# taohan10200/CRA5

Measured on AMD Instinct MI355X. Metric: ERA5 frames/s (721x1440x268) encode+decode, higher is better.
Workload: dtype f32 (3xf16-split MFMA, fp32 accumulate)

## Files before the change

### cra5_amd/config.py

```python
import dataclasses
import os
from dataclasses import dataclass


def _flag(v):
    return str(v).strip().lower() not in ("0", "false", "off", "no", "")


@dataclass
class RuntimeConfig:
    precision: str = "fp32"
    gemm_engine: str = "split"
    attn_engine: str = "split"
    range_guard: bool = True
    gpu_exclusive: bool = True
    gpu_slots: int = 3
    inflight: int = 12
    switch_interval_s: float = 0.0002
    copy_threads: int = 8
    batch_copy_threads: int = 1
    link_serial: bool = True
    numa_bind_single: bool = True
    weights: str = ""

    ENV = {
        "precision": "CRA5_PRECISION", "gemm_engine": "CRA5_GEMM", "attn_engine": "CRA5_ATTN", "range_guard": "CRA5_RANGE_GUARD",
        "gpu_exclusive": "CRA5_GPU_EXCLUSIVE", "gpu_slots": "CRA5_GPU_SLOTS", "inflight": "CRA5_INFLIGHT",
        "switch_interval_s": "CRA5_SWITCH_INTERVAL", "copy_threads": "CRA5_COPY_THREADS",
        "batch_copy_threads": "CRA5_BATCH_COPY_THREADS", "link_serial": "CRA5_LINK_SERIAL",
        "numa_bind_single": "CRA5_NUMA_BIND_SINGLE", "weights": "CRA5_WEIGHTS",
    }

    def __post_init__(self):
        if self.precision not in ("fp32", "f16"):
            raise ValueError("precision (CRA5_PRECISION) must be 'fp32' or 'f16'")
        if self.gemm_engine not in ("split", "f32"):
            raise ValueError("gemm_engine (CRA5_GEMM) must be 'split' or 'f32'")
        if self.attn_engine not in ("split", "f32"):
            raise ValueError("attn_engine (CRA5_ATTN) must be 'split' or 'f32'")
        if self.gpu_slots < 0 or self.inflight < 1 or not (1 <= self.copy_threads <= 64) or not (1 <= self.batch_copy_threads <= 64):
            raise ValueError("gpu_slots >= 0, inflight >= 1, 1 <= copy threads <= 64")
# ... 33 lines not shown
```

### cra5_amd/csrc/elementwise.hip

```cpp
#include <hip/hip_runtime.h>
#include <math.h>

#include "../../include/cra5_amd.h"
#include "split.h"
#pragma clang force_cuda_host_device begin
#include "rans_resolve.h"
#pragma clang force_cuda_host_device end

CRA5_RANGE_TU(elementwise)
#ifdef CRA5_RANGE_CHECK
extern "C" {
int cra5_range_counts_gemm(unsigned long long *, int);
int cra5_range_counts_attn(unsigned long long *, int);
int cra5_range_counts_attn_f32(unsigned long long *, int);
int cra5_range_counts_hyper(unsigned long long *, int);
}
#endif

namespace {

__device__ __forceinline__ float wave_sum(float v) {
#pragma unroll
  for (int off = 32; off > 0; off >>= 1) v += __shfl_xor(v, off, 64);
  return v;
// ... 47 lines not shown
        if (ys_plain) cra5_store_plain4(ys + (size_t)row * 2 * Kp, c, o.x, o.y, o.z, o.w);
        else cra5_store_split4(ys + (size_t)row * 2 * Kp, c, o.x, o.y, o.z, o.w);
      }
    }
  }
  if (ys)
    for (int c = D + lane; c < Kp; c += 64) {
      if (ys_plain) cra5_store_plain(ys + (size_t)row * 2 * Kp, c, 0.f);
      else cra5_store_split(ys + (size_t)row * 2 * Kp, c, 0.f);
    }
}

__global__ __launch_bounds__(256) void im2col_kernel(const float *__restrict__ x, const float *__restrict__ mean,
                                                     const float *__restrict__ stdv, float *__restrict__ cols,
                                                     unsigned short *__restrict__ cols_s, int C, int H, int W,
                                                     int kh, int kw, int sh, int sw, int Hp, int Wp, int ldk, int plain) {
  const int K = C * kh * kw;
  const size_t total = (size_t)Hp * Wp * K;
  for (size_t e = (size_t)blockIdx.x * blockDim.x + threadIdx.x; e < total; e += (size_t)gridDim.x * blockDim.x) {
    const int tok = (int)(e / K);
    const int k = (int)(e - (size_t)tok * K);
    const int ph = tok / Wp, pw = tok - ph * Wp;
    const int c = k / (kh * kw);
    const int ij = k - c * kh * kw;
    const int i = ij / kw, j = ij - i * kw;
    float v = x[((size_t)c * H + (ph * sh + i)) * W + (pw * sw + j)];
    if (mean) v = (v - mean[c]) / stdv[c];
    if (cols) cols[(size_t)tok * ldk + k] = v;
    if (cols_s) {
      if (plain) cra5_store_plain(cols_s + (size_t)tok * 2 * ldk, k, v);
      else cra5_store_split(cols_s + (size_t)tok * 2 * ldk, k, v);
    }
  }
}

__global__ __launch_bounds__(256) void col2im_kernel(const float *__restrict__ cols, const float *__restrict__ mean,
                                                     const float *__restrict__ stdv, float *__restrict__ x, int C,
                                                     int H, int W, int kh, int kw, int sh, int sw, int Hp, int Wp,
                                                     int ldn) {
  const size_t total = (size_t)C * H * W;
  for (size_t e = (size_t)blockIdx.x * blockDim.x + threadIdx.x; e < total; e += (size_t)gridDim.x * blockDim.x) {
    const int col = (int)(e % W);
    const size_t t = e / W;
    const int row = (int)(t % H);
    const int c = (int)(t / H);
// ... 16 lines not shown
    if (mean) acc = acc * stdv[c] + mean[c];
    x[e] = acc;
  }
}


constexpr int TILE_TOK = 16;
constexpr int TILE_CH = 2;
constexpr int TILE_CH_S = 2;
constexpr int IM2COL_GROUP = 2;

template <int KH, int KW>
__global__ __launch_bounds__(256) void im2col_tiled_kernel(const float *__restrict__ x, const float *__restrict__ mean,
                                                           const float *__restrict__ stdv, float *__restrict__ cols,
                                                           unsigned short *__restrict__ cols_s, int C, int H, int W,
                                                           int sh, int Hp, int Wp, int ldk, int plain) {
  constexpr int SEG = TILE_TOK * KW;
  constexpr int TS = TILE_CH * KH * KW + 4;
  static_assert((TILE_CH * KH * KW) % 4 == 0, "a block's K offset must stay 16-byte aligned");
  constexpr int NL = 4;
  static_assert(TILE_CH * KH * (SEG / 4) <= 256 * NL, "a channel chunk must fit one pass of loads");
  __shared__ __attribute__((aligned(16))) float tile[TILE_TOK * TS];
  const int tiles_w = Wp / TILE_TOK;
  const int n_cc = (C + TILE_CH - 1) / TILE_CH;
  constexpr int G = IM2COL_GROUP;
  const int n_g = (n_cc + G - 1) / G;
  const int g = blockIdx.x % n_g;
  const int pwt = (blockIdx.x / n_g) % tiles_w;
  const int ph = blockIdx.x / (n_g * tiles_w);
  const int col0 = pwt * SEG;
  const int cc_lo = g * G, cc_hi = min(cc_lo + G, n_cc);
// ... 27 lines not shown
        for (int u = 0; u < 4; ++u) vv[u] = (vv[u] - m) / sd;
      }
#pragma unroll
      for (int u = 0; u < 4; ++u) {
        const int col = p4 * 4 + u;
        const int t = col / KW, j = col - t * KW;
        tile[t * TS + row * KW + j] = vv[u];
      }
    }
  }
  __syncthreads();
  if (cc + 1 < cc_hi) load(cc + 1);
  const int kpt = nc * KH * KW;
  const int q4 = (kpt + 3) / 4;
  const int kbase = c0 * KH * KW;
  for (int e = threadIdx.x; e < TILE_TOK * q4; e += 256) {
    const int t = e / q4, k4 = (e - t * q4) * 4;
    const float4 v = *reinterpret_cast<const float4 *>(tile + t * TS + k4);
    const size_t tok = (size_t)ph * Wp + pwt * TILE_TOK + t;
    if (k4 + 4 <= kpt) {
      if (cols) *reinterpret_cast<float4 *>(cols + tok * ldk + kbase + k4) = v;
      if (cols_s) {
        if (plain) cra5_store_plain4(cols_s + tok * 2 * ldk, kbase + k4, v.x, v.y, v.z, v.w);
        else cra5_store_split4(cols_s + tok * 2 * ldk, kbase + k4, v.x, v.y, v.z, v.w);
      }
    } else {
      const float vv[4] = {v.x, v.y, v.z, v.w};
      for (int u = 0; k4 + u < kpt; ++u) {
        if (cols) cols[tok * ldk + kbase + k4 + u] = vv[u];
        if (cols_s) {
          if (plain) cra5_store_plain(cols_s + tok * 2 * ldk, kbase + k4 + u, vv[u]);
          else cra5_store_split(cols_s + tok * 2 * ldk, kbase + k4 + u, vv[u]);
        }
      }
    }
  }
  if (plain && cols_s && cc == n_cc - 1) {
    const int K = C * KH * KW, npad = ldk - K;
    for (int e = threadIdx.x; e < TILE_TOK * npad; e += 256) {
      const int t = e / npad, k = K + (e - t * npad);
      cols_s[((size_t)ph * Wp + pwt * TILE_TOK + t) * 2 * ldk + k] = 0;
    }
  }
  if (cc + 1 < cc_hi) __syncthreads();
  }
}

template <int KH, int KW>
__global__ __launch_bounds__(256) void col2im_tiled_kernel(const float *__restrict__ cols, const float *__restrict__ mean,
                                                           const float *__restrict__ stdv, float *__restrict__ x, int C,
                                                           int H, int W, int sh, int Hp, int Wp, int ldn) {
  constexpr int SEG = TILE_TOK * KW;
// ... 381 lines not shown
#define CRA5_LN(V) hipLaunchKernelGGL(layernorm_kernel<V>, grid, block, 0, st, x, ldx, gamma, beta, y, ldy, y_split, split_kp, rows, D, eps, split_plain)
  if (D <= 256) CRA5_LN(1);
  else if (D <= 512) CRA5_LN(2);
  else if (D <= 1024) CRA5_LN(4);
  else CRA5_LN(8);
#undef CRA5_LN
  return (int)hipGetLastError();
}

int cra5_im2col_f32(const float *x, const float *mean, const float *stdv, float *cols, uint16_t *cols_split, int C,
                    int H, int W, int kh, int kw, int sh, int sw, int Hp, int Wp, int ldk, int split_plain, void *stream) {
  if (!x || (!cols && !cols_split) || C <= 0 || ldk < C * kh * kw) return CRA5_ERR_ARG;
  if (cols_split && (ldk % 32)) return CRA5_ERR_ARG;
  if ((Hp - 1) * sh + kh > H || (Wp - 1) * sw + kw > W) return CRA5_ERR_ARG;
  if ((mean == nullptr) != (stdv == nullptr)) return CRA5_ERR_ARG;
  if (kh == 11 && kw == 10 && sw == 10 && sh == 10 && Wp % TILE_TOK == 0 && (W % 4) == 0 && (ldk % 4) == 0 &&
      ((uintptr_t)x & 15) == 0) {
    const int n_cc = (C + TILE_CH - 1) / TILE_CH;
    const int blocks = (Wp / TILE_TOK) * Hp * ((n_cc + IM2COL_GROUP - 1) / IM2COL_GROUP);
    hipLaunchKernelGGL((im2col_tiled_kernel<11, 10>), dim3(blocks), dim3(256), 0, (hipStream_t)stream, x, mean, stdv,
                       cols, cols_split, C, H, W, sh, Hp, Wp, ldk, split_plain);
    return (int)hipGetLastError();
  }
  if (split_plain && ldk != C * kh * kw) return CRA5_ERR_ARG;
  const size_t total = (size_t)Hp * Wp * C * kh * kw;
  hipLaunchKernelGGL(im2col_kernel, dim3(grid_for(total)), dim3(256), 0, (hipStream_t)stream, x, mean, stdv, cols,
                     cols_split, C, H, W, kh, kw, sh, sw, Hp, Wp, ldk, split_plain);
  return (int)hipGetLastError();
}

int cra5_col2im_f32(const float *cols, const float *mean, const float *stdv, float *x, int C, int H, int W, int kh,
                    int kw, int sh, int sw, int Hp, int Wp, int ldn, void *stream) {
  if (!x || !cols || C <= 0 || ldn < C * kh * kw) return CRA5_ERR_ARG;
  if ((Hp - 1) * sh + kh != H || (Wp - 1) * sw + kw != W) return CRA5_ERR_ARG;
  if ((mean == nullptr) != (stdv == nullptr)) return CRA5_ERR_ARG;
  if (kh == 11 && kw == 10 && sw == 10 && sh == 10 && Wp % TILE_TOK == 0 && (W % 4) == 0 && (ldn % 4) == 0 &&
      ((uintptr_t)cols & 15) == 0 && ((uintptr_t)x & 15) == 0) {
    const int blocks = (Wp / TILE_TOK) * Hp * ((C + TILE_CH_S - 1) / TILE_CH_S);
    hipLaunchKernelGGL((col2im_tiled_kernel<11, 10>), dim3(blocks), dim3(256), 0, (hipStream_t)stream, cols, mean,
                       stdv, x, C, H, W, sh, Hp, Wp, ldn);
    return (int)hipGetLastError();
  }
// ... 155 lines not shown
```

### cra5_amd/csrc/gemm_split_f16.hip

```cpp
#include <hip/hip_runtime.h>
#include <stdlib.h>
#include <type_traits>

#include "../../include/cra5_amd.h"
#include "split.h"

CRA5_RANGE_TU(gemm)

typedef float f32x16 __attribute__((ext_vector_type(16)));
typedef _Float16 half8 __attribute__((ext_vector_type(8)));

namespace {

constexpr int BK = 32;

__device__ __forceinline__ float gelu_erf(float x) {
  const float t = __builtin_fabsf(x) * 0.70710678118654752440f;
  const float k = __builtin_amdgcn_rcpf(__builtin_fmaf(0.4f, t, 1.0f));
  float p = 0.03080804832279682f;
  p = __builtin_fmaf(p, k, -0.3524225652217865f);
  p = __builtin_fmaf(p, k, 1.0205539464950562f);
  p = __builtin_fmaf(p, k, -0.7088391780853271f);
  p = __builtin_fmaf(p, k, 0.6733116507530212f);
  p = __builtin_fmaf(p, k, 0.0958886444568634f);
// ... 35 lines not shown
  if (threadIdx.x == 0 && blockIdx.x < 8192) g_gemm_trace[blockIdx.x * 5 + (slot)] = wall_clock64();
#else
#define CRA5_TRACE(slot)
#endif

struct UnembedArgs {
  float *side;
  const float *mean, *stdv;
  int H, W, Hp, Wp;
};

template <int WM, int WN, int TM, int TN, bool LONGK, int NPROD = 3, bool UE = false>
__global__ __launch_bounds__(WM *WN * 64, ((WM * WN == 4 && TM == 3) ? 2 : 1)) void gemm_nt_split_kernel(
    const unsigned short *__restrict__ A, long lda, const unsigned short *__restrict__ W, long ldw, float *C,
    int ldc, unsigned short *Cs, long ldcs, const float *__restrict__ bias, const float *res, int ldr, int M,
    int N, int Kp, float wscale_inv, int flags, int tiles_n, UnembedArgs ue) {
  constexpr int BM = WM * TM * 32;
  constexpr int BN = WN * TN * 32;
  constexpr int NT = WM * WN * 64;
  constexpr int ROWS_PER_PASS = NT / 8;
  constexpr int A_P = BM / ROWS_PER_PASS;
  constexpr int B_P = BN / ROWS_PER_PASS;
  static_assert(BM % ROWS_PER_PASS == 0 && BN % ROWS_PER_PASS == 0, "tile/threads mismatch");
  constexpr int STAGE = (BM + BN) * 64;

  __shared__ __attribute__((aligned(16))) unsigned short lds[2 * STAGE];

  CRA5_TRACE(0);
#ifdef CRA5_GEMM_TRACE
  if (threadIdx.x == 0 && blockIdx.x < 8192) g_gemm_trace[blockIdx.x * 5 + 4] = clock64();
#endif
// ... 53 lines not shown
        src[q] = W + (size_t)min(n0 + row_, N - 1) * ldw + poffs + (size_t)ka * 64;
      if (ASM_DMA)
        soff[q] = (unsigned)((((size_t)(isA ? (size_t)(min(m0 + row_, M - 1) - m0) * lda : (size_t)(min(n0 + row_, N - 1) - n0) * ldw)) + poffs) * 2);
    }
  }
  if (ASM_DMA) {
    curA = reinterpret_cast<unsigned long long>(A + (size_t)m0 * lda) + (unsigned long long)ka * 128;
    curW = reinterpret_cast<unsigned long long>(W + (size_t)n0 * ldw) + (unsigned long long)ka * 128;
  }
#if defined(__HIP_DEVICE_COMPILE__)
#define CRA5_GLDS16(SRC, DST) __builtin_amdgcn_global_load_lds(SRC, DST, 16, 0, 0)
#else
#define CRA5_GLDS16(SRC, DST) (void)(SRC)
#endif
#define CRA5_DMA_KSTRIDE (2 * KSTEP * 2)
  const unsigned kstride_a = a_plain ? 128u : (unsigned)CRA5_DMA_KSTRIDE, kstride_w = w_plain ? 128u : (unsigned)CRA5_DMA_KSTRIDE;
#if defined(__HIP_DEVICE_COMPILE__)
#define CRA5_STAGE_LOAD(BUF)                                                                   \
  {                                                                                            \
    if (ASM_DMA) {                                                                             \
             \
      const unsigned ldsb_ = (unsigned)(size_t)((__attribute__((address_space(3))) unsigned short *)(lds + (BUF)*STAGE)); \
      _Pragma("unroll") for (int q = 0; q < IPW; ++q) {                                        \
        const unsigned dst_ = ldsb_ + (wave_dma + q * NWAVE) * 1024;                           \
        asm volatile("s_mov_b32 m0, %0\n\ts_nop 0\n\tglobal_load_lds_dwordx4 %1, %2"          \
                     :: "s"(dst_), "v"(soff[q]), "s"((q * NWAVE * 8 < BM) ? curA : curW) : "memory", "m0"); \
      }                                                                                        \
      curA += kstride_a;                                                                       \
      curW += kstride_w;                                                                       \
    } else {                                                                                   \
      _Pragma("unroll") for (int q = 0; q < IPW; ++q) {                                        \
// ... 196 lines not shown

__global__ __launch_bounds__(256) void split_rows_kernel(const float *__restrict__ x, long ldx,
                                                         unsigned short *__restrict__ out, int rows, int K, int Kp,
                                                         float scale) {
  const size_t total = (size_t)rows * Kp;
  for (size_t e = (size_t)blockIdx.x * blockDim.x + threadIdx.x; e < total; e += (size_t)gridDim.x * blockDim.x) {
    const int r = (int)(e / Kp), k = (int)(e - (size_t)r * Kp);
    const float v = (k < K) ? x[(size_t)r * ldx + k] * scale : 0.f;
    cra5_store_split(out + (size_t)r * 2 * Kp, k, v);
  }
}

template <int WM, int WN, int TM, int TN, bool LONGK, int NPROD = 3, bool UE = false>
int launch(const unsigned short *A, long lda, const unsigned short *W, long ldw, float *C, int ldc,
           unsigned short *Cs, long ldcs, const float *bias, const float *res, int ldr, int M, int N, int Kp,
           float wscale_inv, int flags, hipStream_t st, UnembedArgs ue = UnembedArgs{}) {
  constexpr int BM = WM * TM * 32, BN = WN * TN * 32;
  const int tiles_m = (M + BM - 1) / BM, tiles_n = (N + BN - 1) / BN;
  hipLaunchKernelGGL((gemm_nt_split_kernel<WM, WN, TM, TN, LONGK, NPROD, UE>), dim3(tiles_m * tiles_n),
                     dim3(WM * WN * 64), 0, st, A, lda, W, ldw, C, ldc, Cs, ldcs, bias, res, ldr, M, N, Kp, wscale_inv,
                     flags, tiles_n, ue);
  return (int)hipGetLastError();
}

__global__ __launch_bounds__(256) void unembed_fixup_kernel(const float *__restrict__ side, const float *__restrict__ mean,
                                                            const float *__restrict__ stdv, float *__restrict__ x, int C,
                                                            int H, int W, int Hp) {
  const int w4 = W / 4;
  const size_t total = (size_t)C * (Hp + 1) * w4;
  for (size_t e = (size_t)blockIdx.x * blockDim.x + threadIdx.x; e < total; e += (size_t)gridDim.x * blockDim.x) {
    const int p4 = (int)(e % w4);
    const size_t t = e / w4;
    const int i = (int)(t % (Hp + 1)), c = (int)(t / (Hp + 1));
    float4 v = make_float4(0.f, 0.f, 0.f, 0.f);
    bool have = false;
    if (i > 0) {
// ... 4 lines not shown
      const float4 b = *reinterpret_cast<const float4 *>(side + (((size_t)c * Hp + i) * 2 + 0) * W + 4 * p4);
      v = have ? make_float4(v.x + b.x, v.y + b.y, v.z + b.z, v.w + b.w) : b;
    }
    if (mean) {
      const float m = mean[c], sd = stdv[c];
      v = make_float4(v.x * sd + m, v.y * sd + m, v.z * sd + m, v.w * sd + m);
    }
    *reinterpret_cast<float4 *>(x + ((size_t)c * H + (size_t)10 * i) * W + 4 * p4) = v;
  }
}

}

static int gemm_dispatch(const unsigned short *A, long lda, const unsigned short *W, long ldw, float *C, int ldc,
                         unsigned short *C_split, long ldcs, const float *bias, const float *res, int ldr, int M,
                         int N, int Kp, float wscale_inv, int flags, hipStream_t st) {
  const long tiles128 = (long)((M + 127) / 128) * ((N + 127) / 128);
#define CRA5_GO(WM, WN, TM, TN, LK) \
  return launch<WM, WN, TM, TN, LK>(A, lda, W, ldw, C, ldc, C_split, ldcs, bias, res, ldr, M, N, Kp, wscale_inv, flags, st)
#ifdef CRA5_GEMM_TRACE
  static const int forced = [] {
    const char *e = getenv("CRA5_GEMM_TILE");
    return e ? atoi(e) : 0;
  }();
#else
  constexpr int forced = 0;
#endif
  const bool longk = Kp > 8192;
  const bool force_wide = flags & CRA5_GEMM_WIDE_K;
  if (force_wide && (!(flags & CRA5_GEMM_HI_ONLY) || longk || (Kp % 64))) return CRA5_ERR_ARG;
  constexpr int PLAIN_ANY = CRA5_GEMM_A_PLAIN | CRA5_GEMM_W_PLAIN | CRA5_GEMM_OUT_PLAIN;
  if ((flags & PLAIN_ANY) && (!(flags & CRA5_GEMM_HI_ONLY) || longk || (tiles128 < 256 && !force_wide) || (Kp % 64)))
    return CRA5_ERR_ARG;
  if (longk) CRA5_GO(2, 2, 2, 2, true);
  if (flags & CRA5_GEMM_HI_ONLY) {
    const bool wide = (M >= 1024 && N >= 2048);
    if (tiles128 < 256 && !force_wide)
      return launch<2, 2, 1, 1, false, 1>(A, lda, W, ldw, C, ldc, C_split, ldcs, bias, res, ldr, M, N, Kp, wscale_inv, flags, st);
    if (Kp % 64 == 0) {
      if (wide)
        return launch<2, 4, 4, 2, false, 2>(A, lda, W, ldw, C, ldc, C_split, ldcs, bias, res, ldr, M, N, Kp, wscale_inv, flags, st);
      return launch<2, 4, 3, 2, false, 2>(A, lda, W, ldw, C, ldc, C_split, ldcs, bias, res, ldr, M, N, Kp, wscale_inv, flags, st);
    }
    if (wide)
      return launch<2, 4, 4, 2, false, 1>(A, lda, W, ldw, C, ldc, C_split, ldcs, bias, res, ldr, M, N, Kp, wscale_inv, flags, st);
    return launch<2, 4, 3, 2, false, 1>(A, lda, W, ldw, C, ldc, C_split, ldcs, bias, res, ldr, M, N, Kp, wscale_inv, flags, st);
  }
  int tile = forced;
  if (!tile) {
    if (tiles128 < 256) tile = 64;
    else if (M >= 1024 && N >= 2048) tile = 256;
    else if (M >= 1024 && N >= 512) tile = 192;
    else tile = 128;
  }
  if (tile == 64) CRA5_GO(2, 2, 1, 1, false);
  if (tile == 192) CRA5_GO(2, 4, 3, 2, false);
  if (tile == 256) CRA5_GO(2, 4, 4, 2, false);
  CRA5_GO(2, 2, 2, 2, false);
#undef CRA5_GO
}

extern "C" int cra5_gemm_nt_split(const uint16_t *A, int lda_kp, const uint16_t *W, int ldw_kp, float *C, int ldc,
                                  uint16_t *C_split, int ldc_split_kp, const float *bias, const float *res, int ldr,
                                  int M, int N, int Kp, float wscale_inv, int flags, void *stream) {
  if (!A || !W || (!C && !C_split) || M <= 0 || N <= 0 || Kp <= 0 || (Kp % BK)) return CRA5_ERR_ARG;
  if (lda_kp < Kp || ldw_kp < Kp || (lda_kp % 32) || (ldw_kp % 32)) return CRA5_ERR_ARG;
  if (lda_kp >= (1 << 21) || ldw_kp >= (1 << 21)) return CRA5_ERR_ARG;
  if (((uintptr_t)A & 15) || ((uintptr_t)W & 15)) return CRA5_ERR_ARG;
  if ((flags & CRA5_EPI_BIAS) && !bias) return CRA5_ERR_ARG;
  if ((flags & CRA5_EPI_RES) && !res) return CRA5_ERR_ARG;
  if (C_split && (ldc_split_kp % 32 || ldc_split_kp < N)) return CRA5_ERR_ARG;
  hipStream_t st = (hipStream_t)stream;
  const bool a_plain = flags & CRA5_GEMM_A_PLAIN, w_plain = flags & CRA5_GEMM_W_PLAIN, o_plain = flags & CRA5_GEMM_OUT_PLAIN;
  const long lda = a_plain ? (long)lda_kp : 2L * lda_kp, ldw = w_plain ? (long)ldw_kp : 2L * ldw_kp;
  const long ldcs = o_plain ? (long)ldc_split_kp : 2L * ldc_split_kp;
  if (Kp > 8192 && C && !C_split && !(flags & CRA5_EPI_GELU)) {
    const int nchunk = (Kp + 8191) / 8192;
    const int gran = ((flags & CRA5_GEMM_HI_ONLY) && Kp % 64 == 0) ? 64 : 32;
    const int per = ((Kp / gran + nchunk - 1) / nchunk) * gran;
    for (int k0 = 0, i = 0; k0 < Kp; k0 += per, ++i) {
      const int kc = (Kp - k0 < per) ? Kp - k0 : per;
      const int f = ((i == 0) ? flags : CRA5_EPI_RES) | (flags & (CRA5_GEMM_HI_ONLY | CRA5_GEMM_A_PLAIN | CRA5_GEMM_W_PLAIN));
      const int rc = gemm_dispatch(A + (a_plain ? 1L : 2L) * k0, lda, W + (w_plain ? 1L : 2L) * k0, ldw, C, ldc, nullptr, 0, (i == 0) ? bias : nullptr,
                                   (i == 0) ? res : C, (i == 0) ? ldr : ldc, M, N, kc, wscale_inv, f, st);
      if (rc) return rc;
    }
    return 0;
  }
  return gemm_dispatch(A, lda, W, ldw, C, ldc, C_split, ldcs, bias, res, ldr, M, N, Kp, wscale_inv, flags, st);
}

extern "C" __attribute__((visibility("hidden"))) int cra5_internal_gemm_split_tile(
    const unsigned short *A, long lda, const unsigned short *W, long ldw, float *C, int ldc, unsigned short *Cs,
    long ldcs, const float *bias, const float *res, int ldr, int M, int N, int Kp, float wscale_inv, int flags,
    int tile, hipStream_t st) {
  if (tile == 64) return launch<2, 2, 1, 1, false>(A, lda, W, ldw, C, ldc, Cs, ldcs, bias, res, ldr, M, N, Kp, wscale_inv, flags, st);
  return launch<2, 2, 2, 2, false>(A, lda, W, ldw, C, ldc, Cs, ldcs, bias, res, ldr, M, N, Kp, wscale_inv, flags, st);
}

extern "C" int cra5_split_f16(const float *x, int ldx, uint16_t *out, int rows, int K, int Kp, float scale,
                              void *stream) {
  if (!x || !out || rows <= 0 || K <= 0 || Kp < K || (Kp % 32)) return CRA5_ERR_ARG;
  size_t total = (size_t)rows * Kp;
  size_t g = (total + 255) / 256;
// ... 65 lines not shown
```

### cra5_amd/ops.py

```python
import contextlib
import ctypes
import os
import threading

import numpy as np
import torch

from ._lib import check, lib

EPI_BIAS, EPI_GELU, EPI_RES, GEMM_HI_ONLY = 1, 2, 4, 8


_TLS = threading.local()


def _stream():
    s = getattr(_TLS, "stream", None)
    if s is not None:
        return s
    return ctypes.c_void_p(torch.cuda.current_stream().cuda_stream)


@contextlib.contextmanager
def stream_scope():
# ... 164 lines not shown
    M, K = a.shape
    N = w.shape[0]
    assert w.shape[1] == K
    if out is None:
        out = torch.empty((M, N), device=a.device, dtype=torch.float32)
    flags = (EPI_BIAS if bias is not None else 0) | (EPI_GELU if gelu else 0) | (EPI_RES if res is not None else 0)
    ev = TIMER.start() if TIMER is not None else None
    check(lib().cra5_gemm_nt_f32(_p(a), _row_stride(a), _p(w), _row_stride(w), _p(out), _row_stride(out), _p(bias),
                                 _p(res), _row_stride(res) if res is not None else 0, M, N, K, flags, _stream()),
          "cra5_gemm_nt_f32")
    if ev is not None:
        TIMER.stop("gemm_nt_f32", ev, 2.0 * M * N * K)
    return out


class SplitMat:

    __slots__ = ("data", "rows", "K", "Kp", "scale_inv", "plain")

    def __init__(self, data, rows, K, Kp, scale_inv=1.0, plain=False):
        self.data, self.rows, self.K, self.Kp, self.scale_inv = data, rows, K, Kp, scale_inv
        self.plain = plain

    @property
    def pitch(self):
        return self.data.shape[1] if self.plain else self.Kp

    def plain_copy(self):
        assert not self.plain
        hi = self.data.view(self.rows, self.Kp // 32, 2, 32)[:, :, 0].reshape(self.rows, self.Kp).contiguous()
        return SplitMat(hi, self.rows, self.K, self.Kp, self.scale_inv, plain=True)

    @staticmethod
    def empty(rows, K, device, zero=False):
        Kp = (K + 31) // 32 * 32
        data = (torch.zeros if zero else torch.empty)((rows, 2 * Kp), device=device, dtype=torch.int16)
        return SplitMat(data, rows, K, Kp)

    def planes(self):
        if self.plain:
            hi = self.data.view(torch.float16)[:, : self.K].float()
            return hi, torch.zeros_like(hi)
        h = self.data.view(torch.float16).view(self.rows, self.Kp // 32, 2, 32).float()
        return (h[:, :, 0].reshape(self.rows, self.Kp)[:, : self.K].contiguous(),
                h[:, :, 1].reshape(self.rows, self.Kp)[:, : self.K].contiguous())

    def to_float(self):
        if self.plain:
            return self.data.view(torch.float16)[:, : self.K].float() * self.scale_inv
        h = self.data.view(torch.float16).view(self.rows, self.Kp // 32, 2, 32).float()
        return ((h[:, :, 0] + h[:, :, 1]).reshape(self.rows, self.Kp)[:, : self.K]) * self.scale_inv


def _devs(*ts):
    for t in ts:
        if t is not None and not t.is_cuda:
            raise RuntimeError("cra5_amd device op called with a non-GPU tensor: the HIP path is the only path")


def split_f16(x, scale_pow2=None, out=None):
    _dev(x)
    rows, K = x.shape
# ... 3 lines not shown
        if amax > 0 and amax == amax and amax != float("inf"):
            import math
            scale = 2.0 ** (12 - math.floor(math.log2(amax)))
    elif scale_pow2 is not None:
        scale = float(scale_pow2)
    if out is None:
        out = SplitMat.empty(rows, K, x.device)
    check(lib().cra5_split_f16(_p(x), _row_stride(x), _p(out.data), rows, K, out.Kp, scale, _stream()),
          "cra5_split_f16")
    out.scale_inv = 1.0 / scale
    out.plain = False
    return out


GEMM_A_PLAIN, GEMM_W_PLAIN, GEMM_OUT_PLAIN, GEMM_WIDE_K = 16, 32, 64, 128


def plain_ok(M, N, Kp):
    return ((M + 127) // 128) * ((N + 127) // 128) >= 256 and Kp % 64 == 0


def gemm_nt_split(a, w, bias=None, res=None, gelu=False, out=None, out_split=None, want_f32=True, hi_only=False,
                  out_plain=False, wide_k=False):
    _devs(a.data, w.data)
    _dev(bias, res, out)
    M, N = a.rows, w.rows
    assert a.Kp == w.Kp and a.K == w.K, (a.K, w.K)
    assert a.scale_inv == 1.0, "activations are split unscaled"
    if out is None and want_f32:
        out = torch.empty((M, N), device=a.data.device, dtype=torch.float32)
    if out_split is not None:
        assert out_split.rows == M and out_split.K == N
    flags = (EPI_BIAS if bias is not None else 0) | (EPI_GELU if gelu else 0) | (EPI_RES if res is not None else 0)
    if hi_only:
        flags |= GEMM_HI_ONLY
    if a.plain or w.plain or out_plain:
        assert hi_only, "plain-f16 operands exist in the reduced-precision mode only"
        flags |= (GEMM_A_PLAIN if a.plain else 0) | (GEMM_W_PLAIN if w.plain else 0) | (GEMM_OUT_PLAIN if out_plain else 0)
    if wide_k:
        assert hi_only, "the 64-wide k-step form exists in the reduced-precision mode only"
        flags |= GEMM_WIDE_K
    if out_split is not None:
        out_split.plain = bool(out_plain)
    ev = TIMER.start() if TIMER is not None else None
    check(lib().cra5_gemm_nt_split(_p(a.data), a.pitch, _p(w.data), w.pitch, _p(out),
                                   _row_stride(out) if out is not None else 0,
                                   _p(out_split.data) if out_split is not None else None,
                                   out_split.pitch if out_split is not None else 0, _p(bias), _p(res),
                                   _row_stride(res) if res is not None else 0, M, N, a.Kp, float(w.scale_inv),
                                   flags, _stream()), "cra5_gemm_nt_split")
    if ev is not None:
        small = ((M + 127) // 128) * ((N + 127) // 128) < 256
        TIMER.stop("gemm_nt_split_small" if small else "gemm_nt_split", ev, 2.0 * M * N * a.K)
    return out


# ... 171 lines not shown
def split_attention_ok(C, heads, wh, ww, H=None, W=None):
    L = wh * ww
    return (C % heads == 0 and C // heads == 64 and L % 32 == 0
            and (L <= MAX_WIN_TOKENS or (wh == H and ww == W)))


def im2col(x, kh, kw, sh, sw, ldk=None, mean=None, std=None, out=None, out_split=None, out_plain=False):
    _dev(x, mean, std, out)
    C, H, W = x.shape
    Hp, Wp = (H - kh) // sh + 1, (W - kw) // sw + 1
    K = C * kh * kw
    assert x.is_contiguous()
    if out_split is not None:
        assert out_split.rows == Hp * Wp and out_split.K == K
        ev = TIMER.start() if TIMER is not None else None
        out_split.plain = bool(out_plain)
        check(lib().cra5_im2col_f32(_p(x), _p(mean), _p(std), None, _p(out_split.data), C, H, W, kh, kw, sh, sw, Hp,
                                    Wp, out_split.Kp, int(bool(out_plain)), _stream()), "cra5_im2col_f32")
        if ev is not None:
            TIMER.stop("im2col", ev, 4.0 * C * H * W + 4.0 * Hp * Wp * K)
        return out_split
    ldk = ldk or K
    if out is None:
        out = torch.zeros((Hp * Wp, ldk), device=x.device, dtype=torch.float32)
    assert out.is_contiguous() and out.shape[1] == ldk
    check(lib().cra5_im2col_f32(_p(x), _p(mean), _p(std), _p(out), None, C, H, W, kh, kw, sh, sw, Hp, Wp, ldk,
                                0, _stream()), "cra5_im2col_f32")
    return out


def col2im(cols, C, kh, kw, sh, sw, Hp, Wp, mean=None, std=None, out=None):
    _dev(cols, mean, std, out)
    H, W = (Hp - 1) * sh + kh, (Wp - 1) * sw + kw
# ... 482 lines not shown
```

### cra5_amd/vaeformer.py

```python
import contextlib
import math
import threading
import time
from collections import OrderedDict

import numpy as np
import torch
import torch.nn as nn

from . import ops, subset
from ._lib import ERR_RANGE, Cra5Error, StreamDesyncError
from .config import RuntimeConfig, runtime_setting
from .entropy import EntropyBottleneck, GaussianConditional, get_scale_table

__all__ = ["VAEformer", "config_for", "block_windows"]



_DD_KW_268 = dict(z_dim=None, learnable_pos=True, window=True, window_size=[(24, 24), (12, 48), (48, 12)], interval=4,
                  drop_path_rate=0., round_padding=True, pad_attn_mask=True,
                  test_pos_mode='learnable_simple_interpolate', lms_checkpoint_train=True, img_size=(721, 1440))
_PRIOR_KW_268 = dict(z_dim=256, embed_dim=360, depth=8, num_heads=5, interval=1, learnable_pos=True, window=False,
                     drop_path_rate=0., round_padding=True, pad_attn_mask=True,
                     test_pos_mode='learnable_simple_interpolate', lms_checkpoint_train=False, img_size=(72, 144))
# ... 232 lines not shown
        self.phase_log = None
        self.host_log = None
        self.f16_layout = "plain"
        self._derived = {}
        self._sub_cache = OrderedDict()
        self._derive_lock = threading.RLock()
        self._gpu_lock = threading.Lock()
        self._fallback_lock = threading.Lock()
        self.fused_unembed = True
        self._gpu_sem = None
        self._tls = threading.local()
        self.eval()

    precision = runtime_setting("precision")
    range_guard = runtime_setting("range_guard")
    gpu_exclusive = runtime_setting("gpu_exclusive")
    gpu_slots = runtime_setting("gpu_slots")

    @property
    def gemm_mode(self):
        o = getattr(self._tls, "engine_override", None)
        return o if o is not None else self.runtime.gemm_engine

    @gemm_mode.setter
    def gemm_mode(self, v):
        self.runtime = self.runtime.replace(gemm_engine=v)

    @property
    def attn_mode(self):
        o = getattr(self._tls, "engine_override", None)
# ... 145 lines not shown
    def _sbuf(self, name, rows, K, zero=False):
        dev = self.device
        return self._cached("split", name, (rows, K, dev), lambda: ops.SplitMat.empty(rows, K, dev, zero=zero))

    def _weight2d(self, key, w):
        if key == "g_s.final":
            return self._derive("w2d." + key, w, lambda w: w.reshape(w.shape[0], -1).t().contiguous())
        return w.detach().reshape(w.shape[0], -1)

    def _wsplit(self, key, w):
        return self._derive("ws." + key, w, lambda w: ops.split_f16(self._weight2d(key, w).contiguous(), "auto"))

    def _wplain(self, key, w):
        return self._derive("wpl." + key, w, lambda _w: self._wsplit(key, w).plain_copy())

    def _hi(self, key):
        return self.precision == "f16" and key.startswith(("g_a.", "g_s."))

    def _plain_gemm(self, key, M, N, K):
        return (self._hi(key) and self.f16_layout == "plain" and self.gemm_mode == "split"
                and ops.plain_ok(M, N, _rup(K, 32)))

    def _wf32(self, key, w, pad32=False):
        w2 = self._weight2d(key, w)
        if pad32 and w2.shape[1] % 32:
            def mk(_):
                out = torch.zeros((w2.shape[0], _rup(w2.shape[1], 32)), device=w2.device, dtype=torch.float32)
                out[:, : w2.shape[1]] = w2
                return out
            return self._derive("wp." + key, w, mk)
# ... 6 lines not shown

    def _ln(self, x, norm, name, plain=False):
        rows, D = x.shape
        if self.gemm_mode == "split":
            sm = self._sbuf(name, rows, D)
            ops.layernorm(x, norm.weight, norm.bias, 1e-6, out_split=sm, want_f32=False, out_plain=plain)
            return sm
        return ops.layernorm(x, norm.weight, norm.bias, 1e-6, out=self._buf(name, (rows, D)))

    def _mm(self, a, key, w, bias=None, res=None, gelu=False, out=None, out_name=None, out_plain=False):
        if self.gemm_mode == "split":
            W = self._wsplit(key, w)
            hi = self._hi(key)
            if self._plain_gemm(key, a.rows, W.rows, W.K):
                W = self._wplain(key, w)
            else:
                assert not a.plain and not out_plain, key
            if out_name is not None:
                sm = self._sbuf(out_name, a.rows, W.rows)
                ops.gemm_nt_split(a, W, bias=bias, res=res, gelu=gelu, out_split=sm, want_f32=False, hi_only=hi,
                                  out_plain=out_plain)
                return sm
            return ops.gemm_nt_split(a, W, bias=bias, res=res, gelu=gelu, out=out, hi_only=hi)
        W = self._wf32(key, w, pad32=(a.shape[1] % 32 == 0 and self._weight2d(key, w).shape[1] != a.shape[1]))
        if out_name is not None:
            out = self._buf(out_name, (a.shape[0], W.shape[0]))
        return ops.gemm_nt(a, W, bias=bias, res=res, gelu=gelu, out=out)

    def _block(self, blk, pre, t_in, t_out, grid):
        N, D = t_in.shape
# ... 28 lines not shown
        self._mm(att, pre + ".attn.proj", blk.attn.proj.weight, bias=blk.attn.proj.bias, res=t_in, out=t_out)
        h = self._ln(t_out, blk.norm2, f"h{D}", plain=fused_attn and p_fc1)
        hid = self._mm(h, pre + ".mlp.fc1", blk.mlp.fc1.weight, bias=blk.mlp.fc1.bias, gelu=True,
                       out_name=f"hid{D}", out_plain=fused_attn and p_fc1 and p_fc2)
        self._mm(hid, pre + ".mlp.fc2", blk.mlp.fc2.weight, bias=blk.mlp.fc2.bias, res=t_out, out=t_out)
        return t_out

    def _encode_y_frame(self, x, mean=None, std=None):
        cfg = self.cfg
        D, L = cfg['embed_dim'], cfg['latent_dim']
        N = self.Hp * self.Wp
        kh, kw = cfg['patch_size']
        sh, sw = cfg['patch_stride']
        K = cfg['in_chans'] * kh * kw
        x = x.contiguous()
        if self.gemm_mode == "split":
            cols = self._sbuf("pe_cols", N, K, zero=True)
            p_pe = (kh, kw, sh, sw) == (11, 10, 10, 10) and self.Wp % 16 == 0 and \
                self._plain_gemm("g_a.patch_embed.proj", N, D, K)
            ops.im2col(x, kh, kw, sh, sw, mean=mean, std=std, out_split=cols, out_plain=p_pe)
        else:
            cols = self._buf("pe_cols", (N, _rup(K, 32)), zero=True)
            ops.im2col(x, kh, kw, sh, sw, ldk=cols.shape[1], mean=mean, std=std, out=cols)
        t = self._buf(f"t{D}", (N, D))
        self._mm(cols, "g_a.patch_embed.proj", self.g_a.patch_embed.proj.weight, bias=self.g_a.patch_embed.proj.bias,
                 res=self.g_a.pos_embed[0], out=t)
        blocks = self.g_a.blocks
        grid = (self.Hp, self.Wp)
        nb = len(blocks)
        for i in range(nb - 2):
            self._block(blocks[i], f"g_a.blocks.{i}", t, t, grid)
# ... 720 lines not shown
```

### include/cra5_amd.h

```cpp
#ifndef CRA5_AMD_H
#define CRA5_AMD_H

#include <stddef.h>
#include <stdint.h>

#ifdef __cplusplus
extern "C" {
#endif

#define CRA5_OK 0
#define CRA5_ERR_ALLOC (-1)
#define CRA5_ERR_INDEX (-2)
#define CRA5_ERR_PMF_DOMAIN (-3)
#define CRA5_ERR_PMF_ZERO (-4)
#define CRA5_ERR_PMF_STEAL (-5)
#define CRA5_ERR_STREAM (-6)
#define CRA5_ERR_ARG (-7)
#define CRA5_ERR_UNAVAILABLE (-8)
#define CRA5_ERR_RANGE (-9)
#define CRA5_ERR_DESYNC (-10)

int cra5_abi_version(void);


// ... 40 lines not shown
                                    int n_cdfs, int cdf_stride, const int32_t *cdf_sizes,
                                    const int32_t *offsets, int32_t *out);
void cra5_rans_decoder_free(void *dec);

int cra5_pmf_to_quantized_cdf(const float *pmf, int n, int precision, uint32_t *cdf);


#define CRA5_EPI_BIAS 1
#define CRA5_EPI_GELU 2
#define CRA5_EPI_RES 4
#define CRA5_GEMM_HI_ONLY 8
#define CRA5_GEMM_A_PLAIN 16
#define CRA5_GEMM_W_PLAIN 32
#define CRA5_GEMM_OUT_PLAIN 64
#define CRA5_GEMM_WIDE_K 128
int cra5_gemm_nt_f32(const float *A, int lda, const float *W, int ldw, float *C, int ldc,
                     const float *bias, const float *res, int ldr, int M, int N, int K,
                     int flags, void *stream);

int cra5_gemm_nt_split(const uint16_t *A, int lda_kp, const uint16_t *W, int ldw_kp, float *C,
                       int ldc, uint16_t *C_split, int ldc_split_kp, const float *bias,
                       const float *res, int ldr, int M, int N, int Kp, float wscale_inv,
                       int flags, void *stream);


int cra5_split_f16(const float *x, int ldx, uint16_t *out, int rows, int K, int Kp, float scale,
                   void *stream);

int cra5_layernorm_f32(const float *x, int ldx, const float *gamma, const float *beta, float *y,
                       int ldy, uint16_t *y_split, int split_kp, int rows, int D, float eps,
// ... 132 lines not shown
```

Before: 30.67.

## Store patch-embed im2col columns and weights in K-panel layout for split GEMM

Adds a K-panel layout in which each 32-wide K block of the split f16 operand is stored as a contiguous [rows x 64] panel. im2col writes directly into this layout and the patch-embed GEMM reads it with a per-k-step stride, with weights converted once and cached. The aim is to make the very long-K (K≈268*110) patch-embed GEMM's loads contiguous per k-step, instead of striding across huge row pitches. The cost is extra flags, validation and kernel parameters, and the tile choice is forced to 192 or 256 for this path.

```diff
diff --git a/cra5_amd/config.py b/cra5_amd/config.py
--- a/cra5_amd/config.py
+++ b/cra5_amd/config.py
@@ -13,6 +13,7 @@
     gemm_engine: str = "split"
     attn_engine: str = "split"
     range_guard: bool = True
+    patch_panels: bool = True
     gpu_exclusive: bool = True
     gpu_slots: int = 3
     inflight: int = 12
@@ -25,6 +26,7 @@
 
     ENV = {
         "precision": "CRA5_PRECISION", "gemm_engine": "CRA5_GEMM", "attn_engine": "CRA5_ATTN", "range_guard": "CRA5_RANGE_GUARD",
+        "patch_panels": "CRA5_PATCH_PANELS",
         "gpu_exclusive": "CRA5_GPU_EXCLUSIVE", "gpu_slots": "CRA5_GPU_SLOTS", "inflight": "CRA5_INFLIGHT",
         "switch_interval_s": "CRA5_SWITCH_INTERVAL", "copy_threads": "CRA5_COPY_THREADS",
         "batch_copy_threads": "CRA5_BATCH_COPY_THREADS", "link_serial": "CRA5_LINK_SERIAL",
diff --git a/cra5_amd/csrc/elementwise.hip b/cra5_amd/csrc/elementwise.hip
--- a/cra5_amd/csrc/elementwise.hip
+++ b/cra5_amd/csrc/elementwise.hip
@@ -85,12 +85,18 @@
 __global__ __launch_bounds__(256) void im2col_kernel(const float *__restrict__ x, const float *__restrict__ mean,
                                                      const float *__restrict__ stdv, float *__restrict__ cols,
                                                      unsigned short *__restrict__ cols_s, int C, int H, int W,
-                                                     int kh, int kw, int sh, int sw, int Hp, int Wp, int ldk, int plain) {
+                                                     int kh, int kw, int sh, int sw, int Hp, int Wp, int ldk, int plain,
+                                                     int Rp) {
   const int K = C * kh * kw;
-  const size_t total = (size_t)Hp * Wp * K;
+  const int Kl = (plain == 2) ? ldk : K;
+  const size_t total = (size_t)Hp * Wp * Kl;
   for (size_t e = (size_t)blockIdx.x * blockDim.x + threadIdx.x; e < total; e += (size_t)gridDim.x * blockDim.x) {
-    const int tok = (int)(e / K);
-    const int k = (int)(e - (size_t)tok * K);
+    const int tok = (int)(e / Kl);
+    const int k = (int)(e - (size_t)tok * Kl);
+    if (k >= K) {
+      cra5_store_split(cols_s + ((size_t)(k >> 5) * Rp + tok) * 64, k & 31, 0.f);
+      continue;
+    }
     const int ph = tok / Wp, pw = tok - ph * Wp;
     const int c = k / (kh * kw);
     const int ij = k - c * kh * kw;
@@ -99,7 +105,8 @@
     if (mean) v = (v - mean[c]) / stdv[c];
     if (cols) cols[(size_t)tok * ldk + k] = v;
     if (cols_s) {
-      if (plain) cra5_store_plain(cols_s + (size_t)tok * 2 * ldk, k, v);
+      if (plain == 2) cra5_store_split(cols_s + ((size_t)(k >> 5) * Rp + tok) * 64, k & 31, v);
+      else if (plain) cra5_store_plain(cols_s + (size_t)tok * 2 * ldk, k, v);
       else cra5_store_split(cols_s + (size_t)tok * 2 * ldk, k, v);
     }
   }
@@ -146,7 +153,7 @@
 __global__ __launch_bounds__(256) void im2col_tiled_kernel(const float *__restrict__ x, const float *__restrict__ mean,
                                                            const float *__restrict__ stdv, float *__restrict__ cols,
                                                            unsigned short *__restrict__ cols_s, int C, int H, int W,
-                                                           int sh, int Hp, int Wp, int ldk, int plain) {
+                                                           int sh, int Hp, int Wp, int ldk, int plain, int Rp) {
   constexpr int SEG = TILE_TOK * KW;
   constexpr int TS = TILE_CH * KH * KW + 4;
   static_assert((TILE_CH * KH * KW) % 4 == 0, "a block's K offset must stay 16-byte aligned");
@@ -204,6 +211,24 @@
   const int kpt = nc * KH * KW;
   const int q4 = (kpt + 3) / 4;
   const int kbase = c0 * KH * KW;
+  if (plain == 2) {
+    const int kend = (cc == n_cc - 1) ? ldk : kbase + kpt;
+    const int kb_lo = kbase >> 5, nkb = ((kend - 1) >> 5) - kb_lo + 1;
+    for (int e = threadIdx.x; e < nkb * (TILE_TOK * 8); e += 256) {
+      const int kb = kb_lo + e / (TILE_TOK * 8), t = (e / 8) % TILE_TOK, q = e & 7;
+      const int k = kb * 32 + q * 4;
+      if (k < kbase || k >= kend) continue;
+      const int rel = k - kbase;
+      const size_t tok = (size_t)ph * Wp + pwt * TILE_TOK + t;
+      unsigned short *chunk = cols_s + ((size_t)kb * Rp + tok) * 64;
+      if (rel + 4 <= kpt) {
+        const float4 v = *reinterpret_cast<const float4 *>(tile + t * TS + rel);
+        cra5_store_split4(chunk, q * 4, v.x, v.y, v.z, v.w);
+      } else {
+        for (int u = 0; u < 4; ++u) cra5_store_split(chunk, q * 4 + u, (rel + u < kpt) ? tile[t * TS + rel + u] : 0.f);
+      }
+    }
+  } else
   for (int e = threadIdx.x; e < TILE_TOK * q4; e += 256) {
     const int t = e / q4, k4 = (e - t * q4) * 4;
     const float4 v = *reinterpret_cast<const float4 *>(tile + t * TS + k4);
@@ -225,7 +250,7 @@
       }
     }
   }
-  if (plain && cols_s && cc == n_cc - 1) {
+  if (plain == 1 && cols_s && cc == n_cc - 1) {
     const int K = C * KH * KW, npad = ldk - K;
     for (int e = threadIdx.x; e < TILE_TOK * npad; e += 256) {
       const int t = e / npad, k = K + (e - t * npad);
@@ -637,18 +662,21 @@
   if (cols_split && (ldk % 32)) return CRA5_ERR_ARG;
   if ((Hp - 1) * sh + kh > H || (Wp - 1) * sw + kw > W) return CRA5_ERR_ARG;
   if ((mean == nullptr) != (stdv == nullptr)) return CRA5_ERR_ARG;
+  if (split_plain == 2 && (!cols_split || cols)) return CRA5_ERR_ARG;
+  split_plain = (split_plain == 2) ? 2 : (split_plain != 0);
+  const int Rp = CRA5_KPANEL_ROWS(Hp * Wp);
   if (kh == 11 && kw == 10 && sw == 10 && sh == 10 && Wp % TILE_TOK == 0 && (W % 4) == 0 && (ldk % 4) == 0 &&
       ((uintptr_t)x & 15) == 0) {
     const int n_cc = (C + TILE_CH - 1) / TILE_CH;
     const int blocks = (Wp / TILE_TOK) * Hp * ((n_cc + IM2COL_GROUP - 1) / IM2COL_GROUP);
     hipLaunchKernelGGL((im2col_tiled_kernel<11, 10>), dim3(blocks), dim3(256), 0, (hipStream_t)stream, x, mean, stdv,
-                       cols, cols_split, C, H, W, sh, Hp, Wp, ldk, split_plain);
+                       cols, cols_split, C, H, W, sh, Hp, Wp, ldk, split_plain, Rp);
     return (int)hipGetLastError();
   }
-  if (split_plain && ldk != C * kh * kw) return CRA5_ERR_ARG;
-  const size_t total = (size_t)Hp * Wp * C * kh * kw;
+  if (split_plain == 1 && ldk != C * kh * kw) return CRA5_ERR_ARG;
+  const size_t total = (size_t)Hp * Wp * ((split_plain == 2) ? ldk : C * kh * kw);
   hipLaunchKernelGGL(im2col_kernel, dim3(grid_for(total)), dim3(256), 0, (hipStream_t)stream, x, mean, stdv, cols,
-                     cols_split, C, H, W, kh, kw, sh, sw, Hp, Wp, ldk, split_plain);
+                     cols_split, C, H, W, kh, kw, sh, sw, Hp, Wp, ldk, split_plain, Rp);
   return (int)hipGetLastError();
 }
 
diff --git a/cra5_amd/csrc/gemm_split_f16.hip b/cra5_amd/csrc/gemm_split_f16.hip
--- a/cra5_amd/csrc/gemm_split_f16.hip
+++ b/cra5_amd/csrc/gemm_split_f16.hip
@@ -73,7 +73,7 @@
 __global__ __launch_bounds__(WM *WN * 64, ((WM * WN == 4 && TM == 3) ? 2 : 1)) void gemm_nt_split_kernel(
     const unsigned short *__restrict__ A, long lda, const unsigned short *__restrict__ W, long ldw, float *C,
     int ldc, unsigned short *Cs, long ldcs, const float *__restrict__ bias, const float *res, int ldr, int M,
-    int N, int Kp, float wscale_inv, int flags, int tiles_n, UnembedArgs ue) {
+    int N, int Kp, float wscale_inv, int flags, int tiles_n, UnembedArgs ue, long ksa, long ksw) {
   constexpr int BM = WM * TM * 32;
   constexpr int BN = WN * TN * 32;
   constexpr int NT = WM * WN * 64;
@@ -157,7 +157,8 @@
 #define CRA5_GLDS16(SRC, DST) (void)(SRC)
 #endif
 #define CRA5_DMA_KSTRIDE (2 * KSTEP * 2)
-  const unsigned kstride_a = a_plain ? 128u : (unsigned)CRA5_DMA_KSTRIDE, kstride_w = w_plain ? 128u : (unsigned)CRA5_DMA_KSTRIDE;
+  const unsigned long long kstride_a = ksa ? (unsigned long long)ksa : (a_plain ? 128ull : (unsigned long long)CRA5_DMA_KSTRIDE);
+  const unsigned long long kstride_w = ksw ? (unsigned long long)ksw : (w_plain ? 128ull : (unsigned long long)CRA5_DMA_KSTRIDE);
 #if defined(__HIP_DEVICE_COMPILE__)
 #define CRA5_STAGE_LOAD(BUF)                                                                   \
   {                                                                                            \
@@ -384,12 +385,12 @@
 template <int WM, int WN, int TM, int TN, bool LONGK, int NPROD = 3, bool UE = false>
 int launch(const unsigned short *A, long lda, const unsigned short *W, long ldw, float *C, int ldc,
            unsigned short *Cs, long ldcs, const float *bias, const float *res, int ldr, int M, int N, int Kp,
-           float wscale_inv, int flags, hipStream_t st, UnembedArgs ue = UnembedArgs{}) {
+           float wscale_inv, int flags, hipStream_t st, UnembedArgs ue = UnembedArgs{}, long ksa = 0, long ksw = 0) {
   constexpr int BM = WM * TM * 32, BN = WN * TN * 32;
   const int tiles_m = (M + BM - 1) / BM, tiles_n = (N + BN - 1) / BN;
   hipLaunchKernelGGL((gemm_nt_split_kernel<WM, WN, TM, TN, LONGK, NPROD, UE>), dim3(tiles_m * tiles_n),
                      dim3(WM * WN * 64), 0, st, A, lda, W, ldw, C, ldc, Cs, ldcs, bias, res, ldr, M, N, Kp, wscale_inv,
-                     flags, tiles_n, ue);
+                     flags, tiles_n, ue, ksa, ksw);
   return (int)hipGetLastError();
 }
 
@@ -424,7 +425,7 @@
 
 static int gemm_dispatch(const unsigned short *A, long lda, const unsigned short *W, long ldw, float *C, int ldc,
                          unsigned short *C_split, long ldcs, const float *bias, const float *res, int ldr, int M,
-                         int N, int Kp, float wscale_inv, int flags, hipStream_t st) {
+                         int N, int Kp, float wscale_inv, int flags, hipStream_t st, long ksa = 0, long ksw = 0) {
   const long tiles128 = (long)((M + 127) / 128) * ((N + 127) / 128);
 #define CRA5_GO(WM, WN, TM, TN, LK) \
   return launch<WM, WN, TM, TN, LK>(A, lda, W, ldw, C, ldc, C_split, ldcs, bias, res, ldr, M, N, Kp, wscale_inv, flags, st)
@@ -442,6 +443,8 @@
   constexpr int PLAIN_ANY = CRA5_GEMM_A_PLAIN | CRA5_GEMM_W_PLAIN | CRA5_GEMM_OUT_PLAIN;
   if ((flags & PLAIN_ANY) && (!(flags & CRA5_GEMM_HI_ONLY) || longk || (tiles128 < 256 && !force_wide) || (Kp % 64)))
     return CRA5_ERR_ARG;
+  const bool kpanel = ksa || ksw;
+  if (kpanel && (longk || (flags & CRA5_GEMM_HI_ONLY) || C_split)) return CRA5_ERR_ARG;
   if (longk) CRA5_GO(2, 2, 2, 2, true);
   if (flags & CRA5_GEMM_HI_ONLY) {
     const bool wide = (M >= 1024 && N >= 2048);
@@ -463,9 +466,14 @@
     else if (M >= 1024 && N >= 512) tile = 192;
     else tile = 128;
   }
+  if (kpanel && tile != 192 && tile != 256) tile = (M >= 1024 && N >= 2048) ? 256 : 192;
   if (tile == 64) CRA5_GO(2, 2, 1, 1, false);
-  if (tile == 192) CRA5_GO(2, 4, 3, 2, false);
-  if (tile == 256) CRA5_GO(2, 4, 4, 2, false);
+#define CRA5_GO_KP(WM, WN, TM, TN)                                                                                      \
+  return launch<WM, WN, TM, TN, false>(A, lda, W, ldw, C, ldc, C_split, ldcs, bias, res, ldr, M, N, Kp, wscale_inv, flags, \
+                                       st, UnembedArgs{}, ksa, ksw)
+  if (tile == 192) CRA5_GO_KP(2, 4, 3, 2);
+  if (tile == 256) CRA5_GO_KP(2, 4, 4, 2);
+#undef CRA5_GO_KP
   CRA5_GO(2, 2, 2, 2, false);
 #undef CRA5_GO
 }
@@ -474,7 +482,10 @@
                                   uint16_t *C_split, int ldc_split_kp, const float *bias, const float *res, int ldr,
                                   int M, int N, int Kp, float wscale_inv, int flags, void *stream) {
   if (!A || !W || (!C && !C_split) || M <= 0 || N <= 0 || Kp <= 0 || (Kp % BK)) return CRA5_ERR_ARG;
-  if (lda_kp < Kp || ldw_kp < Kp || (lda_kp % 32) || (ldw_kp % 32)) return CRA5_ERR_ARG;
+  const bool a_kp = flags & CRA5_GEMM_A_KPANEL, w_kp = flags & CRA5_GEMM_W_KPANEL;
+  if ((a_kp && (flags & CRA5_GEMM_A_PLAIN)) || (w_kp && (flags & CRA5_GEMM_W_PLAIN))) return CRA5_ERR_ARG;
+  if (a_kp ? lda_kp < M : (lda_kp < Kp || (lda_kp % 32))) return CRA5_ERR_ARG;
+  if (w_kp ? ldw_kp < N : (ldw_kp < Kp || (ldw_kp % 32))) return CRA5_ERR_ARG;
   if (lda_kp >= (1 << 21) || ldw_kp >= (1 << 21)) return CRA5_ERR_ARG;
   if (((uintptr_t)A & 15) || ((uintptr_t)W & 15)) return CRA5_ERR_ARG;
   if ((flags & CRA5_EPI_BIAS) && !bias) return CRA5_ERR_ARG;
@@ -482,7 +493,9 @@
   if (C_split && (ldc_split_kp % 32 || ldc_split_kp < N)) return CRA5_ERR_ARG;
   hipStream_t st = (hipStream_t)stream;
   const bool a_plain = flags & CRA5_GEMM_A_PLAIN, w_plain = flags & CRA5_GEMM_W_PLAIN, o_plain = flags & CRA5_GEMM_OUT_PLAIN;
-  const long lda = a_plain ? (long)lda_kp : 2L * lda_kp, ldw = w_plain ? (long)ldw_kp : 2L * ldw_kp;
+  const long lda = a_kp ? 64L : a_plain ? (long)lda_kp : 2L * lda_kp, ldw = w_kp ? 64L : w_plain ? (long)ldw_kp : 2L * ldw_kp;
+  const long ksa = a_kp ? 128L * lda_kp : 0, ksw = w_kp ? 128L * ldw_kp : 0;
+  const long ska = a_kp ? 64L * lda_kp : a_plain ? 32L : 64L, skw = w_kp ? 64L * ldw_kp : w_plain ? 32L : 64L;
   const long ldcs = o_plain ? (long)ldc_split_kp : 2L * ldc_split_kp;
   if (Kp > 8192 && C && !C_split && !(flags & CRA5_EPI_GELU)) {
     const int nchunk = (Kp + 8191) / 8192;
@@ -491,13 +504,13 @@
     for (int k0 = 0, i = 0; k0 < Kp; k0 += per, ++i) {
       const int kc = (Kp - k0 < per) ? Kp - k0 : per;
       const int f = ((i == 0) ? flags : CRA5_EPI_RES) | (flags & (CRA5_GEMM_HI_ONLY | CRA5_GEMM_A_PLAIN | CRA5_GEMM_W_PLAIN));
-      const int rc = gemm_dispatch(A + (a_plain ? 1L : 2L) * k0, lda, W + (w_plain ? 1L : 2L) * k0, ldw, C, ldc, nullptr, 0, (i == 0) ? bias : nullptr,
-                                   (i == 0) ? res : C, (i == 0) ? ldr : ldc, M, N, kc, wscale_inv, f, st);
+      const int rc = gemm_dispatch(A + (k0 / 32) * ska, lda, W + (k0 / 32) * skw, ldw, C, ldc, nullptr, 0, (i == 0) ? bias : nullptr,
+                                   (i == 0) ? res : C, (i == 0) ? ldr : ldc, M, N, kc, wscale_inv, f, st, ksa, ksw);
       if (rc) return rc;
     }
     return 0;
   }
-  return gemm_dispatch(A, lda, W, ldw, C, ldc, C_split, ldcs, bias, res, ldr, M, N, Kp, wscale_inv, flags, st);
+  return gemm_dispatch(A, lda, W, ldw, C, ldc, C_split, ldcs, bias, res, ldr, M, N, Kp, wscale_inv, flags, st, ksa, ksw);
 }
 
 extern "C" __attribute__((visibility("hidden"))) int cra5_internal_gemm_split_tile(
diff --git a/cra5_amd/ops.py b/cra5_amd/ops.py
--- a/cra5_amd/ops.py
+++ b/cra5_amd/ops.py
@@ -202,17 +202,71 @@
     return out
 
 
+def kpanel_rows(rows):
+    return (rows + 255) // 256 * 256
+
+
+def kpanel_from_rows(a, Rp=None):
+    rows, w = a.shape
+    assert w % 64 == 0
+    Rp = kpanel_rows(rows) if Rp is None else Rp
+    assert Rp >= rows
+    if isinstance(a, np.ndarray):
+        out = np.zeros((w // 64, Rp, 64), dtype=a.dtype)
+        out[:, :rows] = a.reshape(rows, w // 64, 64).transpose(1, 0, 2)
+        return out
+    out = torch.zeros((w // 64, Rp, 64), device=a.device, dtype=a.dtype)
+    out[:, :rows] = a.reshape(rows, w // 64, 64).permute(1, 0, 2)
+    return out
+
+
+def kpanel_to_rows(p, rows):
+    nkb, Rp, c = p.shape
+    assert c == 64 and rows <= Rp
+    if isinstance(p, np.ndarray):
+        return np.ascontiguousarray(p[:, :rows].transpose(1, 0, 2)).reshape(rows, nkb * 64)
+    return p[:, :rows].permute(1, 0, 2).contiguous().reshape(rows, nkb * 64)
+
+
+def gemm_chain_chunks(Kp, gran=32):
+    if Kp <= 8192:
+        return [(0, Kp)]
+    nchunk = (Kp + 8191) // 8192
+    per = ((Kp // gran + nchunk - 1) // nchunk) * gran
+    return [(k0, min(per, Kp - k0)) for k0 in range(0, Kp, per)]
+
+
+def kpanel_ok(M, N):
+    return ((M + 127) // 128) * ((N + 127) // 128) >= 256 and M >= 1024 and N >= 512
+
+
 class SplitMat:
 
-    __slots__ = ("data", "rows", "K", "Kp", "scale_inv", "plain")
-
-    def __init__(self, data, rows, K, Kp, scale_inv=1.0, plain=False):
+    __slots__ = ("data", "rows", "K", "Kp", "scale_inv", "plain", "panel")
+
+    def __init__(self, data, rows, K, Kp, scale_inv=1.0, plain=False, panel=0):
         self.data, self.rows, self.K, self.Kp, self.scale_inv = data, rows, K, Kp, scale_inv
+        self.panel = panel
         self.plain = plain
 
     @property
     def pitch(self):
-        return self.data.shape[1] if self.plain else self.Kp
+        return self.panel if self.panel else (self.data.shape[1] if self.plain else self.Kp)
+
+    def panel_copy(self):
+        assert not self.plain and not self.panel
+        d = kpanel_from_rows(self.data)
+        return SplitMat(d, self.rows, self.K, self.Kp, self.scale_inv, panel=d.shape[1])
+
+    def row_copy(self):
+        assert self.panel
+        return SplitMat(kpanel_to_rows(self.data, self.rows), self.rows, self.K, self.Kp, self.scale_inv)
+
+    @staticmethod
+    def empty_panel(rows, K, device):
+        Kp = (K + 31) // 32 * 32
+        Rp = kpanel_rows(rows)
+        return SplitMat(torch.zeros((Kp // 32, Rp, 64), device=device, dtype=torch.int16), rows, K, Kp, panel=Rp)
 
     def plain_copy(self):
         assert not self.plain
@@ -226,6 +280,8 @@
         return SplitMat(data, rows, K, Kp)
 
     def planes(self):
+        if self.panel:
+            return self.row_copy().planes()
         if self.plain:
             hi = self.data.view(torch.float16)[:, : self.K].float()
             return hi, torch.zeros_like(hi)
@@ -234,6 +290,8 @@
                 h[:, :, 1].reshape(self.rows, self.Kp)[:, : self.K].contiguous())
 
     def to_float(self):
+        if self.panel:
+            return self.row_copy().to_float()
         if self.plain:
             return self.data.view(torch.float16)[:, : self.K].float() * self.scale_inv
         h = self.data.view(torch.float16).view(self.rows, self.Kp // 32, 2, 32).float()
@@ -267,6 +325,7 @@
 
 
 GEMM_A_PLAIN, GEMM_W_PLAIN, GEMM_OUT_PLAIN, GEMM_WIDE_K = 16, 32, 64, 128
+GEMM_A_KPANEL, GEMM_W_KPANEL = 256, 512
 
 
 def plain_ok(M, N, Kp):
@@ -293,6 +352,7 @@
     if wide_k:
         assert hi_only, "the 64-wide k-step form exists in the reduced-precision mode only"
         flags |= GEMM_WIDE_K
+    flags |= (GEMM_A_KPANEL if a.panel else 0) | (GEMM_W_KPANEL if w.panel else 0)
     if out_split is not None:
         out_split.plain = bool(out_plain)
     ev = TIMER.start() if TIMER is not None else None
@@ -494,9 +554,13 @@
     if out_split is not None:
         assert out_split.rows == Hp * Wp and out_split.K == K
         ev = TIMER.start() if TIMER is not None else None
-        out_split.plain = bool(out_plain)
+        if out_split.panel:
+            assert not out_plain and out_split.panel == kpanel_rows(Hp * Wp)
+        else:
+            out_split.plain = bool(out_plain)
         check(lib().cra5_im2col_f32(_p(x), _p(mean), _p(std), None, _p(out_split.data), C, H, W, kh, kw, sh, sw, Hp,
-                                    Wp, out_split.Kp, int(bool(out_plain)), _stream()), "cra5_im2col_f32")
+                                    Wp, out_split.Kp, 2 if out_split.panel else int(bool(out_plain)), _stream()),
+              "cra5_im2col_f32")
         if ev is not None:
             TIMER.stop("im2col", ev, 4.0 * C * H * W + 4.0 * Hp * Wp * K)
         return out_split
diff --git a/cra5_amd/vaeformer.py b/cra5_amd/vaeformer.py
--- a/cra5_amd/vaeformer.py
+++ b/cra5_amd/vaeformer.py
@@ -270,6 +270,7 @@
 
     precision = runtime_setting("precision")
     range_guard = runtime_setting("range_guard")
+    patch_panels = runtime_setting("patch_panels")
     gpu_exclusive = runtime_setting("gpu_exclusive")
     gpu_slots = runtime_setting("gpu_slots")
 
@@ -445,6 +446,9 @@
     def _wplain(self, key, w):
         return self._derive("wpl." + key, w, lambda _w: self._wsplit(key, w).plain_copy())
 
+    def _wpanel(self, key, w):
+        return self._derive("wkp." + key, w, lambda _w: self._wsplit(key, w).panel_copy())
+
     def _hi(self, key):
         return self.precision == "f16" and key.startswith(("g_a.", "g_s."))
 
@@ -481,6 +485,9 @@
             hi = self._hi(key)
             if self._plain_gemm(key, a.rows, W.rows, W.K):
                 W = self._wplain(key, w)
+            elif a.panel:
+                assert not hi and not out_plain and out_name is None, key
+                W = self._wpanel(key, w)
             else:
                 assert not a.plain and not out_plain, key
             if out_name is not None:
@@ -539,7 +546,11 @@
         sh, sw = cfg['patch_stride']
         K = cfg['in_chans'] * kh * kw
         x = x.contiguous()
-        if self.gemm_mode == "split":
+        if self.gemm_mode == "split" and self.patch_panels and not self._hi("g_a.patch_embed.proj") and ops.kpanel_ok(N, D):
+            dev = self.device
+            cols = self._cached("split", "pe_cols_kp", (N, K, dev), lambda: ops.SplitMat.empty_panel(N, K, dev))
+            ops.im2col(x, kh, kw, sh, sw, mean=mean, std=std, out_split=cols)
+        elif self.gemm_mode == "split":
             cols = self._sbuf("pe_cols", N, K, zero=True)
             p_pe = (kh, kw, sh, sw) == (11, 10, 10, 10) and self.Wp % 16 == 0 and \
                 self._plain_gemm("g_a.patch_embed.proj", N, D, K)
diff --git a/include/cra5_amd.h b/include/cra5_amd.h
--- a/include/cra5_amd.h
+++ b/include/cra5_amd.h
@@ -78,6 +78,9 @@
 #define CRA5_GEMM_W_PLAIN 32
 #define CRA5_GEMM_OUT_PLAIN 64
 #define CRA5_GEMM_WIDE_K 128
+#define CRA5_GEMM_A_KPANEL 256
+#define CRA5_GEMM_W_KPANEL 512
+#define CRA5_KPANEL_ROWS(R) (((R) + 255) / 256 * 256)
 int cra5_gemm_nt_f32(const float *A, int lda, const float *W, int ldw, float *C, int ldc,
                      const float *bias, const float *res, int ldr, int M, int N, int K,
                      int flags, void *stream);
```

After: 30.82 (median of 3 runs). No clear change (+0.5%).
